# brentp/goleft

Measured on AMD Instinct MI355X. Metric: ref bases/sec per-base depth, 30x WGS synthetic, higher is better.
Workload: dtype int32; 1 GPU; synthetic 30x WGS, hg19 contig lengths (3.1 Gb), 150 bp reads; window=1000, min_mapq=1, min_cov=4, total_ref_bases=3095677412, reads_rank0=619135482, cigar_ops_rank0=687232250, canonical_cigar_ops_rank0=0, tiles_on_the_generic_kernel=24, step=gd_compute on the records as they arrived (nothing derived exists), outputs=int32 per-base depth + int64/int32 window sum/min + class runs, tile_positions=4096, lookback=192

## Files before the change

goleft_amd/csrc/gd_sums_stream.hpp:

```cpp
#pragma once

namespace gd {
namespace sums {

constexpr uint32_t NACC = 256;

struct Acc {
    unsigned long long* lds;
    uint32_t kw0;
    int64_t* wsum;
    uint32_t nwin;
};

__device__ __forceinline__ void add_win(const Acc& A, uint32_t k, uint32_t v)
{
    if (v != 0u && k < A.nwin) {
        const uint32_t rel = k - A.kw0;
        if (rel < NACC) atomicAdd(&A.lds[rel], (unsigned long long)v);
        else atomicAdd(reinterpret_cast<unsigned long long*>(&A.wsum[k]), (unsigned long long)v);
    }
}

__device__ __forceinline__ void add_interval_direct(const Acc& A, uint32_t W, uint32_t wm, uint32_t ws, uint32_t s, uint32_t e)
{
    uint32_t k = div_magic(s, wm, ws);
    uint32_t nb = (k + 1u) * W;
    while (s < e) {
        const uint32_t c = (nb < e ? nb : e) - s;
        add_win(A, k, c);
        s += c; ++k; nb += W;
    }
}

constexpr int U = 4;
constexpr uint32_t GROUP = 64u * U;
constexpr uint32_t GPW = 16;
constexpr int SQ_CAP = 256;
#ifndef GD_SUMS_DRAIN_AT
#define GD_SUMS_DRAIN_AT 256
#endif
constexpr int SQ_DRAIN_AT = GD_SUMS_DRAIN_AT;
#ifndef GD_SUMS_WAVES
#define GD_SUMS_WAVES 1
#endif

typedef const __attribute__((address_space(1))) uint32_t* gptr_u32;

__device__ __forceinline__ void drain_queue(const uint4* Q, uint32_t cnt, int lane, gptr_u32 cigar, uint32_t length,
                                         Acc acc, uint32_t W, uint32_t wm, uint32_t ws)
{
    __builtin_amdgcn_wave_barrier();
    for (uint32_t i = (uint32_t)lane; i < cnt; i += 64u) {
        const uint4 it = Q[i];
        if (it.x & 0x80000000u) {
            uint32_t x = it.x & 0x7fffffffu;
            const uint32_t o3[3] = {it.y, it.z, it.w};
#pragma unroll
            for (int k = 0; k < 3; ++k) {
                const uint32_t o = o3[k], ol = o >> 4, op = o & 0xfu;
                if (((0x18du >> op) & 1u) && x < length) {
                    const uint32_t xe = x + ol;
                    if (((0x181u >> op) & 1u) && ol != 0u) add_interval_direct(acc, W, wm, ws, x, xe < length ? xe : length);
                    x = xe;
                }
            }
            continue;
        }
        const int32_t pu = (int32_t)it.x;
        const gptr_u32 ops = cigar + it.y;
        const uint32_t nu = it.z;
        if (pu >= 0) {
            uint32_t x = (uint32_t)pu;
            for (uint32_t k = 0; k < nu && x < length; ++k) {
                const uint32_t o = ops[k], ol = o >> 4;
                const uint32_t op = o & 0xfu;
                if (!((0x18du >> op) & 1u)) continue;
                const uint32_t xe = x + ol;
                if (((0x181u >> op) & 1u) && ol != 0u) add_interval_direct(acc, W, wm, ws, x, xe < length ? xe : length);
                x = xe;
            }
        } else {
            long long x = pu;
            for (uint32_t k = 0; k < nu; ++k) {
                const uint32_t o = ops[k], ol = o >> 4;
                if (!((0x18du >> (o & 0xfu)) & 1u)) continue;
                if ((0x181u >> (o & 0xfu)) & 1u) {
                    const long long e64 = x + (long long)ol;
                    const uint32_t s = x > 0 ? (x < (long long)length ? (uint32_t)x : length) : 0u;
                    const uint32_t e = e64 < (long long)length ? (e64 > 0 ? (uint32_t)e64 : 0u) : length;
                    if (e > s) add_interval_direct(acc, W, wm, ws, s, e);
                }
                x += (long long)ol;
            }
        }
    }
    __builtin_amdgcn_wave_barrier();
}

struct Stage {
    typedef unsigned int v4u __attribute__((ext_vector_type(4)));
    v4u pv, rv;
    uint32_t ob;
    uint32_t obase;
    uint32_t cg[U];
    unsigned int fw0, fw1, mq;
    uint32_t g0;
};

__global__ __launch_bounds__(256, GD_SUMS_WAVES) void gd_sums_stream_kernel(Job job)
{
    __shared__ uint4 s_q[4 * SQ_CAP];
    __shared__ unsigned long long s_acc[4 * NACC];
    const int lane = threadIdx.x & 63;
    const uint32_t unit = blockIdx.x * 4u + (uint32_t)__builtin_amdgcn_readfirstlane((int)(threadIdx.x >> 6));
    if (unit >= job.n_groups) return;
    int ci = 0;
    for (int base = 0; base < job.n_ctgs; base += 64) {
        const int k = base + lane;
        const bool le = k < job.n_ctgs && job.ctgs[k].grp_beg <= unit;
        const int cnt = __popcll(__builtin_amdgcn_ballot_w64(le));
        ci = base + cnt - 1;
        if (cnt < 64) break;
    }
    ci = __builtin_amdgcn_readfirstlane(ci);
    const ContigDev& c = job.ctgs[ci];
    const uint32_t n_reads = c.n_reads;
    const uint32_t length = (uint32_t)c.length;
    const uint32_t W = (uint32_t)job.W, wm = job.w_magic, ws = job.w_shift;
    const uint32_t nwin = div_magic(length - 1u, wm, ws) + 1u;
    int64_t* const wsum = job.win_sum + c.win_off;
    const gptr_u32 off = (gptr_u32)c.off;
    const gptr_u32 cigar = (gptr_u32)c.cigar;
    const int Q_ = job.Q;

    const uint32_t r_first = (unit - c.grp_beg) * (GROUP * GPW);
    uint32_t r_end = r_first + GROUP * GPW;
    r_end = r_end < n_reads ? r_end : n_reads;
    const rsrc_t r_pos = make_rsrc(c.pos + r_first, (r_end - r_first) * 4u);
    const rsrc_t r_rec = make_rsrc(c.off + r_first, (r_end - r_first + 1u) * 4u);
    const rsrc_t r_flag = make_rsrc((const void*)(c.flag + r_first), ((r_end - r_first + 1u) & ~1u) * 2u);
    const rsrc_t r_mapq = make_rsrc((const void*)(c.mapq + r_first), ((r_end - r_first + 3u) & ~3u));

    uint4* const Q = &s_q[(threadIdx.x >> 6) * SQ_CAP];
    uint32_t qn = 0;
    Acc acc;
    acc.lds = &s_acc[(threadIdx.x >> 6) * NACC];
    acc.kw0 = 0;
    acc.wsum = wsum;
    acc.nwin = nwin;
#pragma unroll
    for (uint32_t i = 0; i < NACC; i += 64u) acc.lds[i + (uint32_t)lane] = 0ull;

    auto load_records = [&](Stage& S, uint32_t g) {
        S.pv = __builtin_amdgcn_raw_buffer_load_b128(r_pos, (int)(g - r_first) * 4 + lane * 16, 0, 0);
        S.rv = __builtin_amdgcn_raw_buffer_load_b128(r_rec, (int)(g - r_first) * 4 + lane * 16, 0, 0);
        typedef unsigned int v2u_t __attribute__((ext_vector_type(2)));
        S.g0 = g;
        S.ob = (uint32_t)__builtin_amdgcn_raw_buffer_load_b32(r_rec, (int)(g - r_first) * 4 + lane * 16 + 16, 0, 0);
        const v2u_t fv = __builtin_amdgcn_raw_buffer_load_b64(r_flag, (int)(g - r_first) * 2 + lane * 8, 0, 0);
        S.fw0 = fv.x; S.fw1 = fv.y;
        S.mq = (uint32_t)__builtin_amdgcn_raw_buffer_load_b32(r_mapq, (int)(g - r_first) + lane * 4, 0, 0);
    };
    auto fetch_ops = [&](Stage& S) {
        {
            const uint32_t o[U + 1] = {S.rv.x, S.rv.y, S.rv.z, S.rv.w, S.ob};
            uint32_t n[U];
            bool keep[U];
            const uint32_t fl[U] = {S.fw0 & 0xffffu, S.fw0 >> 16, S.fw1 & 0xffffu, S.fw1 >> 16};
#pragma unroll
            for (int u = 0; u < U; ++u) {
                const bool valid = S.g0 + (uint32_t)lane * U + (uint32_t)u < r_end;
                n[u] = valid ? o[u + 1] - o[u] : 0u;
                keep[u] = ((fl[u] & job.flag_mask) == 0) & ((int)((S.mq >> (8 * u)) & 0xffu) >= Q_) & (n[u] != 0u);
            }
            typedef unsigned int v4u_t __attribute__((ext_vector_type(4)));
            typedef const __attribute__((address_space(1))) v4u_t* gptr_v4;
            const bool four = ((n[0] & n[1] & n[2] & n[3]) == 1u) & ((n[0] | n[1] | n[2] | n[3]) == 1u);
            v4u_t o4 = {0u, 0u, 0u, 0u};
            if (four) o4 = *(gptr_v4)(cigar + o[0]);
            uint32_t c0[U] = {o4.x, o4.y, o4.z, o4.w}, c1[U] = {0u, 0u, 0u, 0u}, c2[U] = {0u, 0u, 0u, 0u};
            const int32_t pq[U] = {(int32_t)S.pv.x, (int32_t)S.pv.y, (int32_t)S.pv.z, (int32_t)S.pv.w};
            uint32_t three = 0;
            if (__builtin_amdgcn_ballot_w64(!four) != 0ull) {
#pragma unroll
                for (int u = 0; u < U; ++u) {
                    const bool t3 = !four & keep[u] & (n[u] == 3u) & (pq[u] >= 0);
                    if (!four & keep[u]) c0[u] = cigar[o[u]];
                    if (!four & keep[u] & ((n[u] == 2u) | t3)) c1[u] = cigar[o[u] + 1u];
                    if (t3) c2[u] = cigar[o[u] + 2u];
                    three |= t3 ? 1u << u : 0u;
                }
            }
            uint32_t odd3 = three;
            while (__builtin_amdgcn_ballot_w64(odd3 != 0u) != 0ull) {
                const bool mine = odd3 != 0u;
                const int u = mine ? __ffs((int)odd3) - 1 : 0;
                const unsigned long long m = __builtin_amdgcn_ballot_w64(mine);
                const uint32_t np = (uint32_t)__popcll(m);
                if (qn + np > (uint32_t)SQ_CAP) break;
                odd3 &= odd3 - 1u;
                if (mine) {
                    const uint32_t rk = qn + __builtin_amdgcn_mbcnt_hi((uint32_t)(m >> 32), __builtin_amdgcn_mbcnt_lo((uint32_t)m, 0u));
                    const uint32_t pu = (uint32_t)(u == 0 ? pq[0] : u == 1 ? pq[1] : u == 2 ? pq[2] : pq[3]);
                    const uint32_t a0 = u == 0 ? c0[0] : u == 1 ? c0[1] : u == 2 ? c0[2] : c0[3];
                    const uint32_t a1 = u == 0 ? c1[0] : u == 1 ? c1[1] : u == 2 ? c1[2] : c1[3];
                    const uint32_t a2 = u == 0 ? c2[0] : u == 1 ? c2[1] : u == 2 ? c2[2] : c2[3];
                    Q[rk] = make_uint4(pu | 0x80000000u, a0, a1, a2);
                }
                qn += np;
            }
            three &= ~odd3;
            uint32_t kb = 0;
#pragma unroll
            for (int u = 0; u < U; ++u) {
                const uint32_t oa = c0[u] & 0xfu, ob2 = c1[u] & 0xfu;
                const bool ca = (0x181u >> oa) & 1u, ka = (0x18du >> oa) & 1u;
                const bool cb = (n[u] == 2u) & (bool)((0x181u >> ob2) & 1u);
                uint32_t eff = 0xffffffffu;
                if (n[u] <= 2u) {
                    if (ca & !cb) eff = c0[u] >> 4;
                    else if (!ka & cb) eff = c1[u] >> 4;
                    else if (!ca & !cb) eff = 0u;
                }
                const bool k = keep[u] & (eff != 0u) & !((three >> u) & 1u);
                S.cg[u] = eff == 0xffffffffu ? eff : eff << 4;
                kb |= k ? 1u << u : 0u;
            }
            S.obase = kb;
        }
    };
    auto work = [&](const Stage& S, uint32_t g0) {
        const int32_t p[U] = {(int32_t)S.pv.x, (int32_t)S.pv.y, (int32_t)S.pv.z, (int32_t)S.pv.w};
        const uint32_t rec[U] = {S.rv.x, S.rv.y, S.rv.z, S.rv.w};
        uint32_t n[U], ex[U];
        bool keep[U];
        {
            const uint32_t oe[U] = {S.rv.y, S.rv.z, S.rv.w, S.ob};
#pragma unroll
            for (int u = 0; u < U; ++u) {
                keep[u] = (S.obase >> u) & 1u;
                n[u] = keep[u] ? oe[u] - rec[u] : 0u;
                ex[u] = rec[u];
            }
        }

        const bool inb = g0 + (uint32_t)lane * U < r_end;
        const uint32_t kb = inb ? div_magic((uint32_t)(p[0] > 0 ? p[0] : 0), wm, ws) : 0xffffffffu;
        const uint32_t nb0 = inb ? (kb + 1u) * W : 0u;
        const uint32_t nb1 = nb0 + W >= nb0 ? nb0 + W : 0xffffffffu;
        const uint32_t nb2 = nb1 + W >= nb1 ? nb1 + W : 0xffffffffu;
        uint32_t a0 = 0, a1 = 0, a2 = 0;
        uint32_t odd = 0;
#pragma unroll
        for (int u = 0; u < U; ++u) {
            const uint32_t len = S.cg[u] >> 4;
            const uint32_t s = p[u] > 0 ? (uint32_t)p[u] : 0u;
            const uint32_t eu = s + len;
            const uint32_t ec = eu < length ? eu : length;
            const bool fits = keep[u] & (S.cg[u] != 0xffffffffu) & (len < (1u << 22)) & (p[u] >= 0) & (ec <= nb2);
            const uint32_t e = fits ? ec : s;
            const uint32_t l1 = s > nb0 ? s : nb0, l2 = s > nb1 ? s : nb1;
            const uint32_t h0 = e < nb0 ? e : nb0, h1 = e < nb1 ? e : nb1;
            a0 += (h0 > s ? h0 : s) - s;
            a1 += (h1 > l1 ? h1 : l1) - l1;
            a2 += (e > l2 ? e : l2) - l2;
            odd |= (keep[u] & !fits) ? 1u << u : 0u;
        }
        while (__builtin_amdgcn_ballot_w64(odd != 0u) != 0ull) {
            const bool mine = odd != 0u;
            const int u = mine ? __ffs((int)odd) - 1 : 0;
            odd &= odd - 1u;
            const unsigned long long m = __builtin_amdgcn_ballot_w64(mine);
            const uint32_t np = (uint32_t)__popcll(m);
            if (qn + np > (uint32_t)SQ_DRAIN_AT) { drain_queue(Q, qn, lane, cigar, length, acc, W, wm, ws); qn = 0; }
            if (mine) {
                const uint32_t rk = qn + __builtin_amdgcn_mbcnt_hi((uint32_t)(m >> 32),
                                             __builtin_amdgcn_mbcnt_lo((uint32_t)m, 0u));
                const int32_t pu = u == 0 ? p[0] : u == 1 ? p[1] : u == 2 ? p[2] : p[3];
                const uint32_t nu = u == 0 ? n[0] : u == 1 ? n[1] : u == 2 ? n[2] : n[3];
                const uint32_t xu = u == 0 ? ex[0] : u == 1 ? ex[1] : u == 2 ? ex[2] : ex[3];
                Q[rk] = make_uint4((uint32_t)pu, xu, nu, 0u);
            }
            qn += np;
        }

        const uint32_t kb_next = (uint32_t)__builtin_amdgcn_update_dpp((int)0xfffffffeu, (int)kb, 0x130, 0xf, 0xf, false);
        const bool tail = inb && (lane == 63 || kb_next != kb);
        const unsigned long long tm = __builtin_amdgcn_ballot_w64(tail);
        const unsigned long long before = tm & ((1ull << lane) - 1ull);
        const int pt = before != 0ull ? 63 - __clzll((long long)before) : 0;
        const uint32_t s0 = (uint32_t)wave_inclusive_scan((int)a0);
        const uint32_t s1 = (uint32_t)wave_inclusive_scan((int)a1);
        const uint32_t s2 = (uint32_t)wave_inclusive_scan((int)a2);
        const uint32_t q0 = (uint32_t)__shfl((int)s0, pt, 64);
        const uint32_t q1 = (uint32_t)__shfl((int)s1, pt, 64);
        const uint32_t q2 = (uint32_t)__shfl((int)s2, pt, 64);
        if (tail) {
            const bool first = before == 0ull;
            add_win(acc, kb, s0 - (first ? 0u : q0));
            add_win(acc, kb + 1u, s1 - (first ? 0u : q1));
            add_win(acc, kb + 2u, s2 - (first ? 0u : q2));
        }
    };

    Stage A, B, C;
    load_records(A, r_first);
    load_records(B, r_first + GROUP);
    {
        const int32_t p0 = __builtin_amdgcn_readfirstlane((int)A.pv.x);
        acc.kw0 = div_magic((uint32_t)(p0 > 0 ? p0 : 0), wm, ws);
    }
    fetch_ops(A);
    for (uint32_t g = r_first; g < r_end; g += 3u * GROUP) {
        load_records(C, g + 2u * GROUP); fetch_ops(B); work(A, g);
        if (g + GROUP >= r_end) break;
        load_records(A, g + 3u * GROUP); fetch_ops(C); work(B, g + GROUP);
        if (g + 2u * GROUP >= r_end) break;
        load_records(B, g + 4u * GROUP); fetch_ops(A); work(C, g + 2u * GROUP);
    }
    if (qn != 0u) drain_queue(Q, qn, lane, cigar, length, acc, W, wm, ws);
    __builtin_amdgcn_wave_barrier();
#pragma unroll
    for (uint32_t i = 0; i < NACC; i += 64u) {
        const unsigned long long v = acc.lds[i + (uint32_t)lane];
        const uint32_t k = acc.kw0 + i + (uint32_t)lane;
        if (v != 0ull && k < nwin) atomicAdd(reinterpret_cast<unsigned long long*>(&wsum[k]), v);
    }
}

}
}
```

Measured before the change: 806.9 billion ref-bases/s.

## Prefetch eight cigar ops per lane via buffer loads split across pipeline stages

Result: no change. 808.7 billion ref-bases/s, median of 2 (+0.2%).

```diff
diff --git a/goleft_amd/csrc/gd_sums_stream.hpp b/goleft_amd/csrc/gd_sums_stream.hpp
--- a/goleft_amd/csrc/gd_sums_stream.hpp
+++ b/goleft_amd/csrc/gd_sums_stream.hpp
@@ -5,10 +5,12 @@
 
 constexpr uint32_t NACC = 256;
 
+typedef __attribute__((address_space(3))) unsigned long long* lds_u64;
+typedef __attribute__((address_space(1))) unsigned long long* glb_u64;
 struct Acc {
-    unsigned long long* lds;
+    lds_u64 lds;
     uint32_t kw0;
-    int64_t* wsum;
+    glb_u64 wsum;
     uint32_t nwin;
 };
 
@@ -16,8 +18,8 @@
 {
     if (v != 0u && k < A.nwin) {
         const uint32_t rel = k - A.kw0;
-        if (rel < NACC) atomicAdd(&A.lds[rel], (unsigned long long)v);
-        else atomicAdd(reinterpret_cast<unsigned long long*>(&A.wsum[k]), (unsigned long long)v);
+        if (rel < NACC) __hip_atomic_fetch_add(A.lds + rel, (unsigned long long)v, __ATOMIC_RELAXED, __HIP_MEMORY_SCOPE_WORKGROUP);
+        else __hip_atomic_fetch_add(A.wsum + k, (unsigned long long)v, __ATOMIC_RELAXED, __HIP_MEMORY_SCOPE_AGENT);
     }
 }
 
@@ -40,6 +42,10 @@
 #define GD_SUMS_DRAIN_AT 256
 #endif
 constexpr int SQ_DRAIN_AT = GD_SUMS_DRAIN_AT;
+static_assert(SQ_DRAIN_AT <= SQ_CAP, "the queue is drained before a round could write past its last slot");
+constexpr int OPS_FETCHED = 8;
+constexpr uint32_t OPS_DESC_MAX = 0x3ffffff0u;
+constexpr uint32_t OPS_NOWHERE = OPS_DESC_MAX * 4u;
 #ifndef GD_SUMS_WAVES
 #define GD_SUMS_WAVES 1
 #endif
@@ -101,6 +107,7 @@
     typedef unsigned int v4u __attribute__((ext_vector_type(4)));
     v4u pv, rv;
     uint32_t ob;
+    v4u q0, q1;
     uint32_t obase;
     uint32_t cg[U];
     unsigned int fw0, fw1, mq;
@@ -140,91 +147,101 @@
     const rsrc_t r_rec = make_rsrc(c.off + r_first, (r_end - r_first + 1u) * 4u);
     const rsrc_t r_flag = make_rsrc((const void*)(c.flag + r_first), ((r_end - r_first + 1u) & ~1u) * 2u);
     const rsrc_t r_mapq = make_rsrc((const void*)(c.mapq + r_first), ((r_end - r_first + 3u) & ~3u));
+    const uint32_t ops_lim = c.n_ops < OPS_DESC_MAX ? c.n_ops : OPS_DESC_MAX;
+    const rsrc_t r_ops = make_rsrc(c.cigar, ops_lim * 4u);
 
     uint4* const Q = &s_q[(threadIdx.x >> 6) * SQ_CAP];
     uint32_t qn = 0;
     Acc acc;
-    acc.lds = &s_acc[(threadIdx.x >> 6) * NACC];
+    acc.lds = (lds_u64)&s_acc[(threadIdx.x >> 6) * NACC];
     acc.kw0 = 0;
-    acc.wsum = wsum;
+    acc.wsum = (glb_u64)wsum;
     acc.nwin = nwin;
 #pragma unroll
     for (uint32_t i = 0; i < NACC; i += 64u) acc.lds[i + (uint32_t)lane] = 0ull;
 
     auto load_records = [&](Stage& S, uint32_t g) {
-        S.pv = __builtin_amdgcn_raw_buffer_load_b128(r_pos, (int)(g - r_first) * 4 + lane * 16, 0, 0);
         S.rv = __builtin_amdgcn_raw_buffer_load_b128(r_rec, (int)(g - r_first) * 4 + lane * 16, 0, 0);
         typedef unsigned int v2u_t __attribute__((ext_vector_type(2)));
         S.g0 = g;
-        S.ob = (uint32_t)__builtin_amdgcn_raw_buffer_load_b32(r_rec, (int)(g - r_first) * 4 + lane * 16 + 16, 0, 0);
         const v2u_t fv = __builtin_amdgcn_raw_buffer_load_b64(r_flag, (int)(g - r_first) * 2 + lane * 8, 0, 0);
         S.fw0 = fv.x; S.fw1 = fv.y;
         S.mq = (uint32_t)__builtin_amdgcn_raw_buffer_load_b32(r_mapq, (int)(g - r_first) + lane * 4, 0, 0);
     };
-    auto fetch_ops = [&](Stage& S) {
+    auto issue_ops = [&](Stage& S) {
+        const uint32_t nx = (uint32_t)__builtin_amdgcn_update_dpp((int)0xffffffffu, (int)S.rv.x, 0x130, 0xf, 0xf, false);
+        const uint32_t m = S.rv.y > S.rv.z ? S.rv.y : S.rv.z, k = S.rv.w > nx ? S.rv.w : nx;
+        const uint32_t oe = m > k ? m : k;
+        const bool near = S.rv.x <= ops_lim;
+        const uint32_t b0 = near ? S.rv.x * 4u : OPS_NOWHERE;
+        const uint32_t b1 = (near & (oe > S.rv.x + 4u)) ? b0 + 16u : OPS_NOWHERE;
+        S.q0 = __builtin_amdgcn_raw_buffer_load_b128(r_ops, (int)b0, 0, 0);
+        S.q1 = __builtin_amdgcn_raw_buffer_load_b128(r_ops, (int)b1, 0, 0);
+        S.pv = __builtin_amdgcn_raw_buffer_load_b128(r_pos, (int)(S.g0 - r_first) * 4 + lane * 16, 0, 0);
+        const uint32_t fl[U] = {S.fw0 & 0xffffu, S.fw0 >> 16, S.fw1 & 0xffffu, S.fw1 >> 16};
+        uint32_t pass = 0;
+#pragma unroll
+        for (int u = 0; u < U; ++u)
+            pass |= (((fl[u] & job.flag_mask) == 0) & ((int)((S.mq >> (8 * u)) & 0xffu) >= Q_)) ? 1u << u : 0u;
+        S.obase = pass;
+    };
+    auto finish_ops = [&](Stage& S, const Stage& N) {
         {
+            S.ob = (uint32_t)__builtin_amdgcn_update_dpp(__builtin_amdgcn_readfirstlane((int)N.rv.x), (int)S.rv.x, 0x130, 0xf, 0xf, false);
             const uint32_t o[U + 1] = {S.rv.x, S.rv.y, S.rv.z, S.rv.w, S.ob};
-            uint32_t n[U];
-            bool keep[U];
-            const uint32_t fl[U] = {S.fw0 & 0xffffu, S.fw0 >> 16, S.fw1 & 0xffffu, S.fw1 >> 16};
+            uint32_t n[U], d[U];
+            bool keep[U], have[U];
+            const uint32_t m = S.rv.x > S.rv.y ? S.rv.x : S.rv.y, k = S.rv.z > S.rv.w ? S.rv.z : S.rv.w;
+            const uint32_t mk = m > k ? m : k;
+            const bool near = (mk > S.ob ? mk : S.ob) <= ops_lim;
 #pragma unroll
             for (int u = 0; u < U; ++u) {
                 const bool valid = S.g0 + (uint32_t)lane * U + (uint32_t)u < r_end;
                 n[u] = valid ? o[u + 1] - o[u] : 0u;
-                keep[u] = ((fl[u] & job.flag_mask) == 0) & ((int)((S.mq >> (8 * u)) & 0xffu) >= Q_) & (n[u] != 0u);
-            }
-            typedef unsigned int v4u_t __attribute__((ext_vector_type(4)));
-            typedef const __attribute__((address_space(1))) v4u_t* gptr_v4;
-            const bool four = ((n[0] & n[1] & n[2] & n[3]) == 1u) & ((n[0] | n[1] | n[2] | n[3]) == 1u);
-            v4u_t o4 = {0u, 0u, 0u, 0u};
-            if (four) o4 = *(gptr_v4)(cigar + o[0]);
-            uint32_t c0[U] = {o4.x, o4.y, o4.z, o4.w}, c1[U] = {0u, 0u, 0u, 0u}, c2[U] = {0u, 0u, 0u, 0u};
-            const int32_t pq[U] = {(int32_t)S.pv.x, (int32_t)S.pv.y, (int32_t)S.pv.z, (int32_t)S.pv.w};
-            uint32_t three = 0;
-            if (__builtin_amdgcn_ballot_w64(!four) != 0ull) {
-#pragma unroll
-                for (int u = 0; u < U; ++u) {
-                    const bool t3 = !four & keep[u] & (n[u] == 3u) & (pq[u] >= 0);
-                    if (!four & keep[u]) c0[u] = cigar[o[u]];
-                    if (!four & keep[u] & ((n[u] == 2u) | t3)) c1[u] = cigar[o[u] + 1u];
-                    if (t3) c2[u] = cigar[o[u] + 2u];
-                    three |= t3 ? 1u << u : 0u;
-                }
-            }
-            uint32_t odd3 = three;
-            while (__builtin_amdgcn_ballot_w64(odd3 != 0u) != 0ull) {
-                const bool mine = odd3 != 0u;
-                const int u = mine ? __ffs((int)odd3) - 1 : 0;
-                const unsigned long long m = __builtin_amdgcn_ballot_w64(mine);
-                const uint32_t np = (uint32_t)__popcll(m);
-                if (qn + np > (uint32_t)SQ_CAP) break;
-                odd3 &= odd3 - 1u;
-                if (mine) {
-                    const uint32_t rk = qn + __builtin_amdgcn_mbcnt_hi((uint32_t)(m >> 32), __builtin_amdgcn_mbcnt_lo((uint32_t)m, 0u));
-                    const uint32_t pu = (uint32_t)(u == 0 ? pq[0] : u == 1 ? pq[1] : u == 2 ? pq[2] : pq[3]);
-                    const uint32_t a0 = u == 0 ? c0[0] : u == 1 ? c0[1] : u == 2 ? c0[2] : c0[3];
-                    const uint32_t a1 = u == 0 ? c1[0] : u == 1 ? c1[1] : u == 2 ? c1[2] : c1[3];
-                    const uint32_t a2 = u == 0 ? c2[0] : u == 1 ? c2[1] : u == 2 ? c2[2] : c2[3];
-                    Q[rk] = make_uint4(pu | 0x80000000u, a0, a1, a2);
-                }
-                qn += np;
-            }
-            three &= ~odd3;
-            uint32_t kb = 0;
+                d[u] = u == 0 ? 0u : d[u - 1] + n[u - 1];
+                keep[u] = (bool)((S.obase >> u) & 1u) & (n[u] != 0u);
+                have[u] = near & (d[u] < (uint32_t)OPS_FETCHED) & (n[u] <= (uint32_t)OPS_FETCHED - d[u]);
+            }
+            const uint32_t r0 = S.q0.x, r1 = S.q0.y, r2 = S.q0.z, r3 = S.q0.w, r4 = S.q1.x, r5 = S.q1.y, r6 = S.q1.z, r7 = S.q1.w;
+            static_assert(OPS_FETCHED == 8, "pick3 shifts eight ops");
+            auto pick3 = [&](uint32_t i, uint32_t& a, uint32_t& b, uint32_t& c) {
+                const bool s4 = i & 4u, s2 = i & 2u, s1 = i & 1u;
+                const uint32_t t0 = s4 ? r4 : r0, t1 = s4 ? r5 : r1, t2 = s4 ? r6 : r2, t3 = s4 ? r7 : r3, t4 = s4 ? 0u : r4, t5 = s4 ? 0u : r5;
+                const uint32_t v0 = s2 ? t2 : t0, v1 = s2 ? t3 : t1, v2 = s2 ? t4 : t2, v3 = s2 ? t5 : t3;
+                a = s1 ? v1 : v0; b = s1 ? v2 : v1; c = s1 ? v3 : v2;
+            };
+            uint32_t kb = 0, t_u = 0xffffffffu, t_p = 0, t_a = 0, t_b = 0, t_c = 0;
 #pragma unroll
             for (int u = 0; u < U; ++u) {
-                const uint32_t oa = c0[u] & 0xfu, ob2 = c1[u] & 0xfu;
+                uint32_t c0 = r0, c1 = r1, c2 = r2;
+                if (u != 0) pick3(d[u], c0, c1, c2);
+                const uint32_t oa = c0 & 0xfu, ob2 = c1 & 0xfu;
                 const bool ca = (0x181u >> oa) & 1u, ka = (0x18du >> oa) & 1u;
                 const bool cb = (n[u] == 2u) & (bool)((0x181u >> ob2) & 1u);
                 uint32_t eff = 0xffffffffu;
-                if (n[u] <= 2u) {
-                    if (ca & !cb) eff = c0[u] >> 4;
-                    else if (!ka & cb) eff = c1[u] >> 4;
+                if (have[u] & (n[u] <= 2u)) {
+                    if (ca & !cb) eff = c0 >> 4;
+                    else if (!ka & cb) eff = c1 >> 4;
                     else if (!ca & !cb) eff = 0u;
                 }
-                const bool k = keep[u] & (eff != 0u) & !((three >> u) & 1u);
                 S.cg[u] = eff == 0xffffffffu ? eff : eff << 4;
-                kb |= k ? 1u << u : 0u;
+                kb |= (keep[u] & (eff != 0u)) ? 1u << u : 0u;
+                const bool t3 = have[u] & keep[u] & (n[u] == 3u) & ((int32_t)S.pv[u] >= 0) & (t_u == 0xffffffffu);
+                t_u = t3 ? (uint32_t)u : t_u; t_p = t3 ? S.pv[u] : t_p;
+                t_a = t3 ? c0 : t_a; t_b = t3 ? c1 : t_b; t_c = t3 ? c2 : t_c;
+            }
+            {
+                const bool mine = t_u != 0xffffffffu;
+                const unsigned long long m = __builtin_amdgcn_ballot_w64(mine);
+                const uint32_t np = (uint32_t)__popcll(m);
+                if (np != 0u && qn + np <= (uint32_t)SQ_CAP) {
+                    if (mine) {
+                        const uint32_t rk = qn + __builtin_amdgcn_mbcnt_hi((uint32_t)(m >> 32), __builtin_amdgcn_mbcnt_lo((uint32_t)m, 0u));
+                        Q[rk] = make_uint4(t_p | 0x80000000u, t_a, t_b, t_c);
+                        kb &= ~(1u << t_u);
+                    }
+                    qn += np;
+                }
             }
             S.obase = kb;
         }
@@ -306,17 +323,17 @@
     Stage A, B, C;
     load_records(A, r_first);
     load_records(B, r_first + GROUP);
+    issue_ops(A);
     {
         const int32_t p0 = __builtin_amdgcn_readfirstlane((int)A.pv.x);
         acc.kw0 = div_magic((uint32_t)(p0 > 0 ? p0 : 0), wm, ws);
     }
-    fetch_ops(A);
     for (uint32_t g = r_first; g < r_end; g += 3u * GROUP) {
-        load_records(C, g + 2u * GROUP); fetch_ops(B); work(A, g);
+        load_records(C, g + 2u * GROUP); finish_ops(A, B); issue_ops(B); work(A, g);
         if (g + GROUP >= r_end) break;
-        load_records(A, g + 3u * GROUP); fetch_ops(C); work(B, g + GROUP);
+        load_records(A, g + 3u * GROUP); finish_ops(B, C); issue_ops(C); work(B, g + GROUP);
         if (g + 2u * GROUP >= r_end) break;
-        load_records(B, g + 4u * GROUP); fetch_ops(A); work(C, g + 2u * GROUP);
+        load_records(B, g + 4u * GROUP); finish_ops(C, A); issue_ops(A); work(C, g + 2u * GROUP);
     }
     if (qn != 0u) drain_queue(Q, qn, lane, cigar, length, acc, W, wm, ws);
     __builtin_amdgcn_wave_barrier();
@@ -324,9 +341,9 @@
     for (uint32_t i = 0; i < NACC; i += 64u) {
         const unsigned long long v = acc.lds[i + (uint32_t)lane];
         const uint32_t k = acc.kw0 + i + (uint32_t)lane;
-        if (v != 0ull && k < nwin) atomicAdd(reinterpret_cast<unsigned long long*>(&wsum[k]), v);
-    }
-}
-
-}
-}
+        if (v != 0ull && k < nwin) __hip_atomic_fetch_add(acc.wsum + k, v, __ATOMIC_RELAXED, __HIP_MEMORY_SCOPE_AGENT);
+    }
+}
+
+}
+}
```
